# ExaScience/bpmf

Hardware: AMD Instinct MI355X
Metric: user+item column samples/sec per Gibbs iter; test RMSE vs reference (higher is better)
Workload: dtype f64

## Files before the change

bpmf_amd/csrc/kernels.h:

```cpp
#pragma once
#include <hip/hip_runtime.h>
#include <stdint.h>

#include "philox.h"
#include "args.h"

namespace bpmf {

typedef double d4 __attribute__((ext_vector_type(4)));

__device__ __forceinline__ d4 mfma16(double a, double b, d4 c)
{
    return __builtin_amdgcn_mfma_f64_16x16x4f64(a, b, c, 0, 0, 0);
}

__device__ __forceinline__ double mfma44(double a, double b, double c)
{
    return __builtin_amdgcn_mfma_f64_4x4x4f64(a, b, c, 0, 0, 0);
}

template <int K>
struct Rot44 {
    static constexpr int NT = K / 16;
    __host__ __device__ static constexpr int nrot(int TI, int TJ) { return TI == TJ ? 3 : 4; }
    __host__ __device__ static constexpr int aoff(int TI, int TJ)
    {
        int n = 0;
        for (int a = 0; a < NT; ++a)
            for (int b = a; b < NT; ++b) {
                if (a == TI && b == TJ) return n;
                n += nrot(a, b);
            }
        return n;
    }
    static constexpr int NACC = aoff(NT - 1, NT - 1) + 3;
};

template <int D>
__device__ __forceinline__ double quad_rot(double x)
{
    constexpr int CTRL = 0x120 + (16 - 4 * D);
    const long long v = __builtin_bit_cast(long long, x);
    const int lo = __builtin_amdgcn_update_dpp(0, (int)v, CTRL, 0xF, 0xF, true);
    const int hi = __builtin_amdgcn_update_dpp(0, (int)(v >> 32), CTRL, 0xF, 0xF, true);
    return __builtin_bit_cast(double, ((long long)hi << 32) | (unsigned int)lo);
}

template <int K>
__device__ __forceinline__ void rot44_contract(const double (&yy)[K / 16], double (&C)[Rot44<K>::NACC])
{
    using G = Rot44<K>;
    constexpr int NT = K / 16;
    double rot[NT][3];
#pragma unroll
    for (int t = 0; t < NT; ++t) {
        rot[t][0] = yy[t];
        rot[t][1] = quad_rot<1>(yy[t]);
        rot[t][2] = quad_rot<2>(yy[t]);
    }
#pragma unroll
    for (int TI = 0; TI < NT; ++TI)
#pragma unroll
        for (int TJ = TI; TJ < NT; ++TJ)
#pragma unroll
            for (int d = 0; d < G::nrot(TI, TJ); ++d) {
                if (d < 3) C[G::aoff(TI, TJ) + d] = mfma44(yy[TI], rot[TJ][d], C[G::aoff(TI, TJ) + d]);
                else C[G::aoff(TI, TJ) + d] = mfma44(rot[TI][1], yy[TJ], C[G::aoff(TI, TJ) + d]);
            }
}

template <int K, typename Sink>
__device__ __forceinline__ void rot44_images(const double (&C)[Rot44<K>::NACC], double *buf0, double *buf1, int lane, Sink &&sink)
{
    using G = Rot44<K>;
    constexpr int NT = G::NT;
    const int i = lane >> 4, b = (lane >> 2) & 3, j = lane & 3;
    int tix = 0;
#pragma unroll
    for (int TI = 0; TI < NT; ++TI)
#pragma unroll
        for (int TJ = TI; TJ < NT; ++TJ, ++tix) {
            double *img = (tix & 1) ? buf1 : buf0;
#pragma unroll
            for (int d = 0; d < G::nrot(TI, TJ); ++d) {
                const int row = d < 3 ? 4 * b + i : 4 * ((b + 1) & 3) + i, col = d < 3 ? 4 * ((b + d) & 3) + j : 4 * b + j;
                const double v = C[G::aoff(TI, TJ) + d];
                img[row * 16 + col] = v;
                if (TI == TJ && d > 0) img[col * 16 + row] = v;
            }
            __syncthreads();
#pragma unroll
            for (int m = 0; m < 4; ++m) sink(tix, TI, TJ, m, img[(4 * m + i) * 16 + (lane & 15)]);
            __syncthreads();
        }
}

__device__ __forceinline__ double rsqrt_nr(double d)
{
    const double y0 = __builtin_amdgcn_rsq(d);
    const double e = fma(-d, y0 * y0, 1.0);
    const double q = e * fma(0.375, e, 0.5);
    return fma(y0, q, y0);
}

__device__ __forceinline__ double gbcast(double v, int base_bytes, int off)
{
    const int lo = __builtin_amdgcn_ds_bpermute(base_bytes + 4 * off, __double2loint(v));
    const int hi = __builtin_amdgcn_ds_bpermute(base_bytes + 4 * off, __double2hiint(v));
    return __hiloint2double(hi, lo);
}

__device__ __forceinline__ double bcast(double v, int src)
{
    const int lo = __builtin_amdgcn_readlane(__double2loint(v), src);
    const int hi = __builtin_amdgcn_readlane(__double2hiint(v), src);
    return __hiloint2double(hi, lo);
}


__device__ __forceinline__ double polar_r2(double x, double y)
{
#pragma clang fp contract(off)
    return x * x + y * y;
}

__device__ __forceinline__ uint32_t sample_counter(int64_t idx, int ktrue, uint32_t iter_plus_1)
{
    return (uint32_t)((uint64_t)(idx + 1) * (uint64_t)ktrue * (uint64_t)iter_plus_1);
}

#define BPMF_RLX_SYSTEM_ __ATOMIC_RELAXED, __HIP_MEMORY_SCOPE_SYSTEM
enum { BPMF_TMO_GATE = 1, BPMF_TMO_PARAMS = 2, BPMF_TMO_STATS = 3 };
__device__ __forceinline__ void flag_timeout(unsigned long long *tmo, unsigned long long what)
{
    if (tmo) __hip_atomic_store(tmo, what, BPMF_RLX_SYSTEM_);
}

__device__ __forceinline__ void wait_params(const SampleArgs &a)
{
    if (a.gate_flag == nullptr) return;
    const unsigned long long t0 = wall_clock64();
    const unsigned long long limit = a.wait_ticks + (a.wait_ticks >> 1);
    while ((unsigned)__builtin_amdgcn_readfirstlane((int)__hip_atomic_load(a.gate_flag, __ATOMIC_RELAXED, __HIP_MEMORY_SCOPE_AGENT)) != a.gate_want) {
        __builtin_amdgcn_s_sleep(8);
        if (wall_clock64() - t0 > limit) {
            if (threadIdx.x == 0) flag_timeout(a.tmo, BPMF_TMO_PARAMS);
            break;
        }
    }
    asm volatile("" ::: "memory");
}

#ifndef BPMF_PROFILING
#define BPMF_PROFILING 0
#endif
constexpr bool kProfiling = BPMF_PROFILING != 0;
__device__ __forceinline__ uint32_t ablate_bits(const SampleArgs &a)
{
    if constexpr (kProfiling) return a.ablate;
    else return 0u;
}

__device__ __forceinline__ void stamp(const SampleArgs &a, int w, int slot)
{
    if constexpr (!kProfiling) {
        __builtin_amdgcn_sched_barrier(0);
        return;
    }
    if (a.stamps == nullptr || threadIdx.x != 0) return;
    const int probe = (w == 0) ? 0 : ((w == a.nwork / 2) ? 1 : -1);
    if (probe >= 0 && slot < 64) a.stamps[probe * 64 + slot] = wall_clock64();
}

__device__ __forceinline__ int rank_below(unsigned long long m)
{
    return (int)__builtin_amdgcn_mbcnt_hi((unsigned)(m >> 32), __builtin_amdgcn_mbcnt_lo((unsigned)m, 0u));
}

template <int NMAX>
__device__ __forceinline__ void draw_normals(uint32_t counter, int n, double *out_lds, int lane, int pad_to = 0)
{
    for (int i = n + lane; i < pad_to; i += 64) out_lds[i] = 0.0;
    int produced = 0;
    uint32_t base = 0;
    while (produced < n) {
        const Philox4 b = stream_block(counter, base + (uint32_t)lane);
        const double x = 2.0 * canonical53(b.w[3], b.w[2]) - 1.0;
        const double y = 2.0 * canonical53(b.w[1], b.w[0]) - 1.0;
        const double r2 = polar_r2(x, y);
        const bool acc = !(r2 > 1.0 || r2 == 0.0);
        const unsigned long long m = __ballot(acc);
        const int rank = produced + rank_below(m);
        if (acc && rank < n) {
            out_lds[rank] = y * polar_mult(r2);
        }
        produced += __popcll(m);
        base += 64u;
    }
}

template <int NMAX>
__device__ __forceinline__ void draw_normals_deferred(uint32_t counter, int n, double *out_lds, double *r2_lds, int lane, int pad_to = 0)
{
    for (int i = n + lane; i < pad_to; i += 64) out_lds[i] = 0.0;
    int produced = 0;
    uint32_t base = 0;
    while (produced < n) {
        const Philox4 b = stream_block(counter, base + (uint32_t)lane);
        const double x = 2.0 * canonical53(b.w[3], b.w[2]) - 1.0;
        const double y = 2.0 * canonical53(b.w[1], b.w[0]) - 1.0;
        const double r2 = polar_r2(x, y);
        const bool acc = !(r2 > 1.0 || r2 == 0.0);
        const unsigned long long m = __ballot(acc);
        const int rank = produced + rank_below(m);
        if (acc && rank < n) { out_lds[rank] = y; r2_lds[rank] = r2; }
        produced += __popcll(m);
        base += 64u;
    }
    for (int i = lane; i < n; i += 64) {
        const double r2 = r2_lds[i];
        out_lds[i] = out_lds[i] * polar_mult(r2);
    }
}

template <int NMAX>
__device__ __forceinline__ void draw_normals_pair(uint32_t counterA, uint32_t counterB, int n, double *outA, double *outB,
                                                  double *r2A, double *r2B, int lane, int pad_to = 0)
{
    for (int i = n + lane; i < pad_to; i += 64) { outA[i] = 0.0; outB[i] = 0.0; }
    auto attempt = [&](uint32_t counter, uint32_t block, double &y, double &r2) -> bool {
        const Philox4 b = stream_block(counter, block);
        const double x = 2.0 * canonical53(b.w[3], b.w[2]) - 1.0;
        y = 2.0 * canonical53(b.w[1], b.w[0]) - 1.0;
        r2 = polar_r2(x, y);
        return !(r2 > 1.0 || r2 == 0.0);
    };
    int prodA, prodB;
    {
        double y, r2;
        bool acc = attempt(counterA, (uint32_t)lane, y, r2);
        unsigned long long m = __ballot(acc);
        int rank = rank_below(m);
        if (acc && rank < n) { outA[rank] = y; r2A[rank] = r2; }
        prodA = __popcll(m);
        acc = attempt(counterB, (uint32_t)lane, y, r2);
        m = __ballot(acc);
        rank = rank_below(m);
        if (acc && rank < n) { outB[rank] = y; r2B[rank] = r2; }
        prodB = __popcll(m);
    }
    const bool hi = lane >= 32;
    const int l32 = lane & 31;
    uint32_t base = 64u;
    while (prodA < n || prodB < n) {
        double y, r2;
        const bool acc = attempt(hi ? counterB : counterA, base + (uint32_t)l32, y, r2);
        const unsigned long long m = __ballot(acc);
        const unsigned mA = (unsigned)m, mB = (unsigned)(m >> 32);
        const int rank = hi ? prodB + (int)__builtin_amdgcn_mbcnt_hi(mB, 0u) : prodA + (int)__builtin_amdgcn_mbcnt_lo(mA, 0u);
        if (acc && rank < n) { (hi ? outB : outA)[rank] = y; (hi ? r2B : r2A)[rank] = r2; }
        prodA += __popc(mA); prodB += __popc(mB);
        base += 32u;
    }
    for (int i = lane; i < n; i += 64) {
        const double ra = r2A[i], rb = r2B[i];
        outA[i] = outA[i] * polar_mult(ra);
        outB[i] = outB[i] * polar_mult(rb);
    }
}

template <int K>
__device__ __forceinline__ void gram_chunk(const int32_t *__restrict__ rowidx, const double *__restrict__ vals, int len,
                                           const double *__restrict__ other, const double *__restrict__ zero_row, double mean, double alpha,
                                           d4 (&acc)[Geo<K>::NTRI], double (&r)[Geo<K>::NT], int lane, int rowmask = -1)
{
    constexpr int NT = Geo<K>::NT;
    const int kq = lane >> 4, li = lane & 15;
    int ri_n = (0 + lane < len) ? rowidx[lane] : -1;
    double wv_n = (0 + lane < len) ? (vals[lane] - mean) * alpha : 0.0;
    for (int b = 0; b < len; b += 64) {
        const int ri = ri_n;
        const double wv = wv_n;
        if (b + 64 < len) {
            const int q = b + 64 + lane;
            ri_n = (q < len) ? rowidx[q] : -1;
            wv_n = (q < len) ? (vals[q] - mean) * alpha : 0.0;
        }
        const int nsteps = (len - b >= 64) ? 16 : (len - b + 3) >> 2;
        double y[4][NT], w[4];
        auto gather = [&](int g, double (&yy)[4][NT], double (&ww)[4]) {
#pragma unroll
            for (int s = 0; s < 4; ++s) {
                const int src = (g * 4 + s) * 4 + kq;
                const int row = __shfl(ri, src);
                ww[s] = __shfl(wv, src);
                const double *col = (row >= 0) ? other + (size_t)(row & rowmask) * K : zero_row;
#pragma unroll
                for (int t = 0; t < NT; ++t) yy[s][t] = col[(t * 16 + li < K) ? t * 16 + li : 0];
            }
        };
        gather(0, y, w);
#pragma unroll
        for (int g = 0; g < 4; ++g) {
            if (g * 4 >= nsteps) break;
            double yn[4][NT], wn[4];
// ... 658 lines not shown
            __hip_atomic_store(flag_host, seq, BPMF_RLX_SYSTEM);
        }
    }
}

template <int K>
constexpr bool kColstatsRot = (K == 64);

template <int K>
__device__ __forceinline__ void colstats_accumulate(const double *__restrict__ items, int64_t b, int64_t e,
                                                    d4 (&acc)[Geo<K>::NTRI], double (&r)[Geo<K>::NT], int lane, double *img,
                                                    const int32_t *__restrict__ list = nullptr, int64_t c0 = 0)
{
    constexpr int NT = Geo<K>::NT;
    constexpr bool ROT = kColstatsRot<K>;
    const int kq = lane >> 4, li = lane & 15;
    double C[ROT ? Rot44<K>::NACC : 1];
#pragma unroll
    for (int t = 0; t < (ROT ? Rot44<K>::NACC : 1); ++t) C[t] = 0.0;
#pragma unroll
    for (int t = 0; t < Geo<K>::NTRI; ++t) acc[t] = d4{0.0, 0.0, 0.0, 0.0};
#pragma unroll
    for (int t = 0; t < NT; ++t) r[t] = 0.0;
    double yn[2][NT];
    int64_t idn[2];
    auto ids = [&](int64_t c, int64_t (&id)[2]) {
#pragma unroll
        for (int s = 0; s < 2; ++s) {
            const int64_t pos = (c + s * 4 + kq < e) ? c + s * 4 + kq : b;
            id[s] = list ? c0 + (int64_t)list[pos] : pos;
        }
    };
    auto fetch = [&](const int64_t (&id)[2], double (&yy)[2][NT]) {
#pragma unroll
        for (int s = 0; s < 2; ++s) {
            const double *x = items + (size_t)id[s] * K;
#pragma unroll
            for (int t = 0; t < NT; ++t) yy[s][t] = x[(t * 16 + li < K) ? t * 16 + li : 0];
        }
    };
    if (b < e) {
        int64_t id0[2];
        ids(b, id0);
        fetch(id0, yn);
        ids((b + 8 < e) ? b + 8 : b, idn);
    }
    for (int64_t c = b; c < e; c += 8) {
        double y[2][NT];
#pragma unroll
        for (int s = 0; s < 2; ++s) {
            const bool ok = c + s * 4 + kq < e;
#pragma unroll
            for (int t = 0; t < NT; ++t) y[s][t] = (ok && (t * 16 + li < K)) ? yn[s][t] : 0.0;
        }
        fetch(idn, yn);
        ids((c + 16 < e) ? c + 16 : b, idn);
#pragma unroll
        for (int s = 0; s < 2; ++s) {
#pragma unroll
            for (int t = 0; t < NT; ++t) r[t] += y[s][t];
            if constexpr (ROT) {
                rot44_contract<K>(y[s], C);
            } else {
                int tri = 0;
#pragma unroll
                for (int I = 0; I < NT; ++I)
#pragma unroll
                    for (int J = I; J < NT; ++J, ++tri) acc[tri] = mfma16(y[s][I], y[s][J], acc[tri]);
            }
        }
    }
    if constexpr (ROT) rot44_images<K>(C, img, img + 256, lane, [&](int tix, int, int, int m, double v) { acc[tix][m] = v; });
#pragma unroll
    for (int t = 0; t < NT; ++t) {
        r[t] += __shfl_xor(r[t], 16);
        r[t] += __shfl_xor(r[t], 32);
    }
}

template <int K>
__device__ __forceinline__ void colstats_body(int w, const double *__restrict__ items, int64_t c0, int64_t c1, int nwaves,
                                              double *partials, const unsigned long long *__restrict__ fail_in,
                                              double *__restrict__ out, unsigned *ticket, unsigned *flag, unsigned seq,
                                              unsigned long long *tmo, unsigned long long wait_ticks, double *img)
{
    constexpr int NT = Geo<K>::NT, NTRI = Geo<K>::NTRI, PART = Geo<K>::PART;
    constexpr int NSUMS = blob::res_sums(K), NSLICE = (NSUMS + 15) / 16, FAILD = blob::res_failD(K), FAIL = blob::res_fail(K);
    const int lane = threadIdx.x;
    const int64_t n = c1 - c0;
    const int64_t per = (((n + nwaves - 1) / nwaves) + 3) & ~(int64_t)3;
    const int64_t b = c0 + w * per;
    const int64_t e = (b + per < c1) ? b + per : c1;

    {
        d4 acc[NTRI];
        double r[NT];
        colstats_accumulate<K>(items, b, e, acc, r, lane, img);
        double *p = partials + (size_t)w * PART;
#pragma unroll
        for (int t = 0; t < NTRI; ++t)
#pragma unroll
            for (int reg = 0; reg < 4; ++reg) __hip_atomic_store(&p[(t * 4 + reg) * 64 + lane], acc[t][reg], BPMF_RLX_AGENT);
        if (lane < 16) {
#pragma unroll
            for (int t = 0; t < NT; ++t) __hip_atomic_store(&p[NTRI * 256 + t * 16 + lane], r[t], BPMF_RLX_AGENT);
        }
    }

    const int nfin = nwaves < NSLICE ? nwaves : NSLICE;
    asm volatile("s_waitcnt vmcnt(0)" ::: "memory");
    unsigned tk = 0;
    if (lane == 0) tk = __hip_atomic_fetch_add(ticket, 1u, BPMF_RLX_AGENT);
    tk = __builtin_amdgcn_readfirstlane(tk);
    if ((int)tk < nwaves - nfin) return;
    const int f = (int)tk - (nwaves - nfin);
    if (lane == 0) {
        const unsigned long long t0 = wall_clock64();
        while (__hip_atomic_load(ticket, BPMF_RLX_AGENT) < (unsigned)nwaves) {
            __builtin_amdgcn_s_sleep(1);
            if (wait_ticks && wall_clock64() - t0 > wait_ticks) { flag_timeout(tmo, BPMF_TMO_STATS); break; }
        }
    }
    __syncthreads();

    const int o = lane & 15, grp = lane >> 4;
    for (int slice = f; slice < NSLICE; slice += nfin) {
        const int eo = slice * 16 + o;
        double s = 0.0;
        if (eo < NSUMS) {
            int off;
            if (eo < K * K) {
                int i = eo % K, j = eo / K;
                if (i > j) { const int t = i; i = j; j = t; }
                const int I = i >> 4, J = j >> 4;
                const int tri = I * NT - (I * (I - 1)) / 2 + (J - I);
                const int ii = i & 15, jj = j & 15;
                off = (tri * 4 + (ii >> 2)) * 64 + (ii & 3) * 16 + jj;
            } else {
                off = NTRI * 256 + (eo - K * K);
            }
            const int pw = (nwaves + 3) >> 2;
            const int w0 = grp * pw, w1 = (w0 + pw < nwaves) ? w0 + pw : nwaves;
            double acc[16];
#pragma unroll
            for (int u = 0; u < 16; ++u) acc[u] = 0.0;
            for (int ww = w0; ww < w1; ww += 16) {
                double v[16];
#pragma unroll
                for (int u = 0; u < 16; ++u)
                    v[u] = __hip_atomic_load(&partials[(size_t)((ww + u < w1) ? ww + u : w0) * PART + off], BPMF_RLX_AGENT);
#pragma unroll
                for (int u = 0; u < 16; ++u) acc[u] += (ww + u < w1) ? v[u] : 0.0;
            }
#pragma unroll
            for (int h = 8; h >= 1; h >>= 1)
#pragma unroll
                for (int u = 0; u < h; ++u) acc[u] += acc[u + h];
            s = acc[0];
        }
        s += __shfl_xor(s, 16);
        s += __shfl_xor(s, 32);
        if (grp == 0 && eo < NSUMS) __hip_atomic_store(&out[eo], s, BPMF_RLX_SYSTEM);
    }
    if (f == 0 && lane == 0) {
        const unsigned long long fw = __hip_atomic_load(fail_in, BPMF_RLX_AGENT);
        __hip_atomic_store(&out[FAILD], (fw == ~0ull) ? 0.0 : (double)(fw + 1ull), BPMF_RLX_SYSTEM);
        __hip_atomic_store(&reinterpret_cast<unsigned long long *>(out)[FAIL], fw, BPMF_RLX_SYSTEM);
    }
    publish_when_last(ticket + 1, (unsigned)nfin, flag, seq, ticket);
}

template <int K>
__global__ __launch_bounds__(64) void k_colstats(const double *__restrict__ items, int64_t c0, int64_t c1, int nwaves,
                                                 double *partials, const unsigned long long *__restrict__ fail_in,
                                                 double *__restrict__ out, unsigned *ticket, unsigned *flag, unsigned seq,
                                                 unsigned long long *tmo, unsigned long long wait_ticks)
{
    __shared__ double img[kColstatsRot<K> ? 512 : 1];
    colstats_body<K>((int)blockIdx.x, items, c0, c1, nwaves, partials, fail_in, out, ticket, flag, seq, tmo, wait_ticks, img);
}

template <int K>
__global__ __launch_bounds__(256) void k_colstats_wg(const double *__restrict__ items, int64_t c0, int64_t c1, int nwg,
                                                    double *partials, const unsigned long long *__restrict__ fail_in,
                                                    double *__restrict__ out, unsigned *ticket, unsigned *flag, unsigned seq,
                                                    unsigned long long *tmo, unsigned long long wait_ticks,
                                                    const int32_t *__restrict__ list, int part0, int ntot, int finish)
{
    constexpr int NT = Geo<K>::NT, NTRI = Geo<K>::NTRI, PART = Geo<K>::PART, NBLK = (PART + 63) / 64, FAILD = blob::res_failD(K), FAIL = blob::res_fail(K);
    __shared__ double red[PART];
    __shared__ double fin[4][64];
    __shared__ unsigned stk;
    const int tid = threadIdx.x, wave = tid >> 6, lane = tid & 63;
    const int64_t n = c1 - c0;
    const int nvw = nwg * 4, vw = (int)blockIdx.x * 4 + wave;
    const int64_t per = (((n + nvw - 1) / nvw) + 3) & ~(int64_t)3;
    const int64_t b = c0 + vw * per;
    const int64_t e = (b + per < c1) ? b + per : c1;
    {
        d4 acc[NTRI];
        double r[NT];
        static_assert(!kColstatsRot<K> || 4 * 512 <= PART, "the four waves' images fit the reduction buffer");
        colstats_accumulate<K>(items, b, e, acc, r, lane, red + 512 * wave, list, 0);
        if (kColstatsRot<K>) __syncthreads();
        for (int src = 1; src < 4; ++src) {
            if (wave == src) {
#pragma unroll
                for (int t = 0; t < NTRI; ++t)
#pragma unroll
                    for (int reg = 0; reg < 4; ++reg) red[(t * 4 + reg) * 64 + lane] = acc[t][reg];
                if (lane < 16) {
#pragma unroll
                    for (int t = 0; t < NT; ++t) red[NTRI * 256 + t * 16 + lane] = r[t];
                }
            }
            __syncthreads();
            if (wave == 0) {
#pragma unroll
                for (int t = 0; t < NTRI; ++t)
#pragma unroll
                    for (int reg = 0; reg < 4; ++reg) acc[t][reg] += red[(t * 4 + reg) * 64 + lane];
#pragma unroll
                for (int t = 0; t < NT; ++t) r[t] += red[NTRI * 256 + t * 16 + (lane & 15)];
            }
            __syncthreads();
        }
        if (wave == 0) {
            double *p = partials + (size_t)(part0 + (int)blockIdx.x) * PART;
#pragma unroll
            for (int t = 0; t < NTRI; ++t)
#pragma unroll
                for (int reg = 0; reg < 4; ++reg) __hip_atomic_store(&p[(t * 4 + reg) * 64 + lane], acc[t][reg], BPMF_RLX_AGENT);
            if (lane < 16) {
#pragma unroll
                for (int t = 0; t < NT; ++t) __hip_atomic_store(&p[NTRI * 256 + t * 16 + lane], r[t], BPMF_RLX_AGENT);
            }
            asm volatile("s_waitcnt vmcnt(0)" ::: "memory");
        }
    }
    if (!finish) return;
    const int nfin = nwg < NBLK ? nwg : NBLK;
    if (tid == 0) stk = __hip_atomic_fetch_add(ticket, 1u, BPMF_RLX_AGENT);
    __syncthreads();
    const unsigned tk = stk;
    if ((int)tk < nwg - nfin) return;
    const int f = (int)tk - (nwg - nfin);
    if (tid == 0) {
        const unsigned long long t0 = wall_clock64();
        while (__hip_atomic_load(ticket, BPMF_RLX_AGENT) < (unsigned)nwg) {
            __builtin_amdgcn_s_sleep(1);
            if (wait_ticks && wall_clock64() - t0 > wait_ticks) { flag_timeout(tmo, BPMF_TMO_STATS); break; }
        }
    }
    __syncthreads();
    const int pw = (ntot + 3) >> 2;
    const int w0 = wave * pw, w1 = (w0 + pw < ntot) ? w0 + pw : ntot;
    for (int blk = f; blk < NBLK; blk += nfin) {
        const int po = blk * 64 + lane;
        const int pc = po < PART ? po : 0;
        double acc[16];
#pragma unroll
        for (int u = 0; u < 16; ++u) acc[u] = 0.0;
        for (int ww = w0; ww < w1; ww += 16) {
            double v[16];
#pragma unroll
            for (int u = 0; u < 16; ++u)
                v[u] = __hip_atomic_load(&partials[(size_t)((ww + u < w1) ? ww + u : w0) * PART + pc], BPMF_RLX_AGENT);
#pragma unroll
            for (int u = 0; u < 16; ++u) acc[u] += (ww + u < w1) ? v[u] : 0.0;
        }
#pragma unroll
        for (int h = 8; h >= 1; h >>= 1)
#pragma unroll
            for (int u = 0; u < h; ++u) acc[u] += acc[u + h];
        fin[wave][lane] = acc[0];
        __syncthreads();
        if (wave == 0 && po < PART) {
            const double sum = ((fin[0][lane] + fin[1][lane]) + fin[2][lane]) + fin[3][lane];
            if (po < NTRI * 256) {
                const int tri = po >> 8, reg = (po >> 6) & 3, ln = po & 63;
                int I = 0, t = tri;
                while (t >= NT - I) { t -= NT - I; ++I; }
                const int J = I + t;
                const int gi = 16 * I + (ln >> 4) + 4 * reg, gj = 16 * J + (ln & 15);
                if (gi < K && gj < K) {
                    __hip_atomic_store(&out[gi + (size_t)gj * K], sum, BPMF_RLX_SYSTEM);
                    if (I != J) __hip_atomic_store(&out[gj + (size_t)gi * K], sum, BPMF_RLX_SYSTEM);
                }
            } else {
                const int el = po - NTRI * 256;
                if (el < K) __hip_atomic_store(&out[K * K + el], sum, BPMF_RLX_SYSTEM);
            }
        }
        __syncthreads();
    }
    if (f == 0 && tid == 0) {
        const unsigned long long fw = *fail_in;
        __hip_atomic_store(&out[FAILD], (fw == ~0ull) ? 0.0 : (double)(fw + 1ull), BPMF_RLX_SYSTEM);
        __hip_atomic_store(&reinterpret_cast<unsigned long long *>(out)[FAIL], fw, BPMF_RLX_SYSTEM);
    }
    publish_when_last(ticket + 1, (unsigned)nfin, flag, seq, ticket);
}

template <int K, int NT = 256, typename T = double>
__global__ __launch_bounds__(NT) void k_predict(const int32_t *__restrict__ tcol, const int32_t *__restrict__ trow,
                                                 const double *__restrict__ tval, int64_t nnz,
                                                 const T *__restrict__ items, const T *__restrict__ other,
                                                 int64_t col_from, double mean, int n, double *__restrict__ pavg,
                                                 double *__restrict__ pm2, double *partial, double *__restrict__ out,
                                                 unsigned *ticket, unsigned *flag, unsigned seq, TwinArgs tw)
{
    __shared__ double red[4][NT / 64];
    __shared__ double fin[4][NT];
    __shared__ unsigned last;
    auto wsum = [](const double (&r)[NT / 64]) { if constexpr (NT == 256) return (r[0] + r[1]) + (r[2] + r[3]); else return r[0]; };
    const int64_t q = (int64_t)blockIdx.x * NT + threadIdx.x;
    double se = 0.0, se_avg = 0.0, se_t = 0.0, se_avg_t = 0.0;
    if (q < nnz) {
        double d0 = 0.0, d1 = 0.0;
        if constexpr (sizeof(T) == 4) {
            const float4 *m = reinterpret_cast<const float4 *>(items + (size_t)(col_from + tcol[q]) * K);
            const float4 *u = reinterpret_cast<const float4 *>(other + (size_t)trow[q] * K);
#pragma unroll 8
            for (int t = 0; t < K / 4; ++t) {
                const float4 x = m[t], y = u[t];
                d0 = fma((double)x.x, (double)y.x, d0);
                d1 = fma((double)x.y, (double)y.y, d1);
                d0 = fma((double)x.z, (double)y.z, d0);
                d1 = fma((double)x.w, (double)y.w, d1);
            }
        } else {
            const double2 *m = reinterpret_cast<const double2 *>(items + (size_t)(col_from + tcol[q]) * K);
            const double2 *u = reinterpret_cast<const double2 *>(other + (size_t)trow[q] * K);
#pragma unroll
            for (int t = 0; t < K / 2; ++t) {
                const double2 a = m[t], b = u[t];
                d0 = fma(a.x, b.x, d0);
                d1 = fma(a.y, b.y, d1);
            }
        }
        const double pred = (d0 + d1) + mean;
        const double v = tval[q];
        se = (v - pred) * (v - pred);
        double avg = pavg[q];
        const double delta = pred - avg;
        avg = (n == 0) ? pred : (avg + delta / n);
        pavg[q] = avg;
        pm2[q] = (n == 0) ? 0.0 : pm2[q] + delta * (pred - avg);
        se_avg = (v - avg) * (v - avg);
        if (tw.perm) {
            const int qt = tw.perm[q];
            const double pred_t = (d0 + d1) + tw.mean;
            se_t = (v - pred_t) * (v - pred_t);
            double avg_t = tw.pavg[qt];
            const double delta_t = pred_t - avg_t;
            avg_t = (n == 0) ? pred_t : (avg_t + delta_t / n);
            tw.pavg[qt] = avg_t;
            tw.pm2[qt] = (n == 0) ? 0.0 : tw.pm2[qt] + delta_t * (pred_t - avg_t);
            se_avg_t = (v - avg_t) * (v - avg_t);
        }
    }
#pragma unroll
    for (int sh = 32; sh >= 1; sh >>= 1) {
        se += __shfl_xor(se, sh);
        se_avg += __shfl_xor(se_avg, sh);
        se_t += __shfl_xor(se_t, sh);
        se_avg_t += __shfl_xor(se_avg_t, sh);
    }
    const int wv = threadIdx.x >> 6;
    if ((threadIdx.x & 63) == 0) { red[0][wv] = se; red[1][wv] = se_avg; red[2][wv] = se_t; red[3][wv] = se_avg_t; }
    __syncthreads();
    if (threadIdx.x == 0) {
        __hip_atomic_store(&partial[2 * blockIdx.x], wsum(red[0]), BPMF_RLX_AGENT);
        __hip_atomic_store(&partial[2 * blockIdx.x + 1], wsum(red[1]), BPMF_RLX_AGENT);
        if (tw.perm) {
            __hip_atomic_store(&tw.partial[2 * blockIdx.x], wsum(red[2]), BPMF_RLX_AGENT);
            __hip_atomic_store(&tw.partial[2 * blockIdx.x + 1], wsum(red[3]), BPMF_RLX_AGENT);
        }
        asm volatile("s_waitcnt vmcnt(0)" ::: "memory");
        const unsigned t = __hip_atomic_fetch_add(ticket, 1u, BPMF_RLX_AGENT);
        last = (t == gridDim.x - 1) ? 1u : 0u;
    }
    __syncthreads();
    if (!last) return;
    {
        const int64_t nblocks = gridDim.x;
        double a = 0.0, b = 0.0, at = 0.0, bt = 0.0;
        for (int64_t w = threadIdx.x; w < nblocks; w += NT) {
            a += __hip_atomic_load(&partial[2 * w], BPMF_RLX_AGENT);
            b += __hip_atomic_load(&partial[2 * w + 1], BPMF_RLX_AGENT);
            if (tw.perm) {
                at += __hip_atomic_load(&tw.partial[2 * w], BPMF_RLX_AGENT);
                bt += __hip_atomic_load(&tw.partial[2 * w + 1], BPMF_RLX_AGENT);
            }
        }
        fin[0][threadIdx.x] = a; fin[1][threadIdx.x] = b; fin[2][threadIdx.x] = at; fin[3][threadIdx.x] = bt;
        __syncthreads();
        for (int st = NT / 2; st >= 1; st >>= 1) {
            if ((int)threadIdx.x < st) {
#pragma unroll
                for (int c = 0; c < 4; ++c) fin[c][threadIdx.x] += fin[c][threadIdx.x + st];
            }
            __syncthreads();
        }
        if (threadIdx.x == 0) {
            __hip_atomic_store(&out[0], fin[0][0], BPMF_RLX_SYSTEM);
            __hip_atomic_store(&out[1], fin[1][0], BPMF_RLX_SYSTEM);
            if (tw.perm) {
                __hip_atomic_store(&tw.out[0], fin[2][0], BPMF_RLX_SYSTEM);
                __hip_atomic_store(&tw.out[1], fin[3][0], BPMF_RLX_SYSTEM);
            }
            __hip_atomic_store(ticket, 0u, BPMF_RLX_AGENT);
            asm volatile("s_waitcnt vmcnt(0)" ::: "memory");
            __hip_atomic_store(flag, seq, BPMF_RLX_SYSTEM);
            if (tw.perm) __hip_atomic_store(tw.flag, tw.seq, BPMF_RLX_SYSTEM);
        }
    }
}

template <int K>
__global__ __launch_bounds__(256) void k_pack_cols(const double *__restrict__ items, const int32_t *__restrict__ cols, int64_t n,
                                                   double *__restrict__ buf)
{
    typedef double dd2 __attribute__((ext_vector_type(2)));
    constexpr int P = K / 2;
    const int64_t i = (int64_t)blockIdx.x * 256 + threadIdx.x;
    if (i >= n * P) return;
    const int64_t c = i / P;
    const int piece = (int)(i % P);
    reinterpret_cast<dd2 *>(buf)[i] = reinterpret_cast<const dd2 *>(items + (size_t)cols[c] * K)[piece];
}

template <int K>
__global__ __launch_bounds__(256) void k_unpack_cols(const double *__restrict__ buf, const int32_t *__restrict__ cols, int64_t n,
                                                     double *__restrict__ items)
{
    typedef double dd2 __attribute__((ext_vector_type(2)));
    constexpr int P = K / 2;
    const int64_t i = (int64_t)blockIdx.x * 256 + threadIdx.x;
    if (i >= n * P) return;
    const int64_t c = i / P;
    const int piece = (int)(i % P);
    reinterpret_cast<dd2 *>(items + (size_t)cols[c] * K)[piece] = reinterpret_cast<const dd2 *>(buf)[i];
}


__device__ __forceinline__ void gate_stage_body(int block, int nblocks, const unsigned *gate_host, unsigned want, const double *src_host,
                                                double *__restrict__ dst, int n, unsigned *dflag, unsigned dval,
                                                unsigned long long *tmo, unsigned long long wait_ticks)
{
    const int lane = threadIdx.x;
    if (lane == 0) {
        const unsigned long long t0 = wall_clock64();
        int polls = 0;
        while (__hip_atomic_load(gate_host, __ATOMIC_RELAXED, __HIP_MEMORY_SCOPE_SYSTEM) != want) {
            if (polls < 16) { __builtin_amdgcn_s_sleep(4); ++polls; }
            else __builtin_amdgcn_s_sleep(127);
            if (wall_clock64() - t0 > wait_ticks) { flag_timeout(tmo, BPMF_TMO_GATE); break; }
        }
        (void)__hip_atomic_load(gate_host, __ATOMIC_ACQUIRE, __HIP_MEMORY_SCOPE_SYSTEM);
    }
    __syncthreads();
    typedef double d2 __attribute__((ext_vector_type(2)));
    const d2 *src = reinterpret_cast<const d2 *>(src_host);
    d2 *out = reinterpret_cast<d2 *>(dst);
    const int n2 = n >> 1;
    for (int base = block * 256; base < n2; base += 256 * nblocks) {
        d2 v[4];
#pragma unroll
        for (int u = 0; u < 4; ++u) {
            const int i = base + u * 64 + lane;
            v[u] = (i < n2) ? __builtin_nontemporal_load(src + i) : d2{0.0, 0.0};
        }
#pragma unroll
        for (int u = 0; u < 4; ++u) {
            const int i = base + u * 64 + lane;
            if (i < n2) {
                if (dflag) {
                    __hip_atomic_store(dst + 2 * i, v[u].x, BPMF_RLX_AGENT);
                    __hip_atomic_store(dst + 2 * i + 1, v[u].y, BPMF_RLX_AGENT);
                } else {
                    out[i] = v[u];
                }
            }
        }
    }
    if (dflag) {
        asm volatile("s_waitcnt vmcnt(0)" ::: "memory");
        __syncthreads();
        if (lane == 0) __hip_atomic_store(dflag, dval, BPMF_RLX_AGENT);
    }
}



}
```

bpmf_amd/csrc/kernels_wg2.h:

```cpp
#pragma once
#include <type_traits>
#include "kernels_f32.h"
#include "kernels_slab.h"

namespace bpmf {

template <int B, int E, typename F>
__device__ __forceinline__ void static_for(F &&f)
{
    if constexpr (B < E) {
        f(std::integral_constant<int, B>{});
        static_for<B + 1, E>(f);
    }
}

template <int K>
struct GeoW2 {
    using F = GeoF<K>;
    static constexpr int NT = F::NT;
    template <typename T = float> static constexpr size_t lds_bytes() { return (size_t)K * 8 + ((size_t)F::RWORDS + K + 16 + 4) * sizeof(T); }
    static constexpr int PART_FLOATS = F::NTRI * 256 + NT * 16;
};

template <int NT, int NW>
struct FactOwner {
    static_assert(NT == 8 && (NW == 2 || NW == 4), "K = 128");
    __host__ __device__ static constexpr int of(int I, int J)
    {
        if (NW == 2) return 1;
        constexpr int tab[8][8] = {{0, 1, 3, 3, 2, 1, 2, 1}, {0, 1, 2, 1, 1, 2, 3, 3}, {0, 0, 2, 3, 1, 2, 1, 3}, {0, 0, 0, 3, 1, 2, 2, 3},
                                   {0, 0, 0, 0, 1, 2, 3, 1}, {0, 0, 0, 0, 0, 2, 3, 2}, {0, 0, 0, 0, 0, 0, 3, 1}, {0, 0, 0, 0, 0, 0, 0, 1}};
        return tab[I][J];
    }
    __host__ __device__ static constexpr int slot(int I, int J)
    {
        int n = 0;
        for (int i = 1; i < NT; ++i)
            for (int j = i; j < NT; ++j) {
                if (i == I && j == J) return n;
                if (of(i, j) == of(I, J)) ++n;
            }
        return n;
    }
    __host__ __device__ static constexpr int count(int W)
    {
        int n = 0;
        for (int i = 1; i < NT; ++i)
            for (int j = i; j < NT; ++j) n += of(i, j) == W;
        return n;
    }
    __host__ __device__ static constexpr int tiles() { int m = 0; for (int w = 1; w < NW; ++w) m = count(w) > m ? count(w) : m; return m; }
};

template <int MIDBAR = -1>
__device__ __forceinline__ void diag16_factor_invert(double (&A)[4], double (&E)[4], int lane)
{
    const int kq = lane >> 4, x = lane & 3, c16 = lane & 15;
    const W44Select wsel(kq, x);
#pragma unroll
    for (int I = 0; I < 4; ++I) E[I] = (4 * I + kq == c16) ? 1.0 : 0.0;
#pragma unroll
    for (int s = 0; s < 4; ++s) {
        const double dblk = A[s];
        const double d00 = bcast(dblk, 4 * s + 0), d01 = bcast(dblk, 4 * s + 1), d02 = bcast(dblk, 4 * s + 2), d03 = bcast(dblk, 4 * s + 3),
                     d11 = bcast(dblk, 16 + 4 * s + 1), d12 = bcast(dblk, 16 + 4 * s + 2), d13 = bcast(dblk, 16 + 4 * s + 3),
                     d22 = bcast(dblk, 32 + 4 * s + 2), d23 = bcast(dblk, 32 + 4 * s + 3), d33 = bcast(dblk, 48 + 4 * s + 3);
        double WA;
        factor_block44(d00, d01, d02, d03, d11, d12, d13, d22, d23, d33, wsel, WA);
        A[s] = mfma44(WA, A[s], 0.0);
        E[s] = mfma44(WA, E[s], 0.0);
        if (s == MIDBAR) __syncthreads();
        if (s == 3) break;
        double n1 = 0.0, n2 = 0.0, n3 = 0.0;
        if (s < 1) n1 = -quad_splat<1>(A[s]);
        if (s < 2) n2 = -quad_splat<2>(A[s]);
        n3 = -quad_splat<3>(A[s]);
        if (s < 1) { A[1] = mfma44(n1, A[s], A[1]); E[1] = mfma44(n1, E[s], E[1]); }
        if (s < 2) { A[2] = mfma44(n2, A[s], A[2]); E[2] = mfma44(n2, E[s], E[2]); }
        A[3] = mfma44(n3, A[s], A[3]); E[3] = mfma44(n3, E[s], E[3]);
    }
}

template <int K, int NW, int W, typename T = float>
__device__ __forceinline__ void wg2_column(const SampleArgs &a, int w, unsigned char *smem, int tid)
{
    using G = GeoF<K>;
    using X = WgTraits<T>;
    typedef typename X::acc_t acc_t;
    constexpr bool F32 = sizeof(T) == 4;
    constexpr int NT = G::NT, TPW = (G::NTRI + NW - 1) / NW;
    double *zs = reinterpret_cast<double *>(smem);
    T *R = reinterpret_cast<T *>(zs + K);
    T *bv = R + G::RWORDS, *xs = bv, *ts = bv + K;
    unsigned *sticket = reinterpret_cast<unsigned *>(ts + 16);
    const int lane = tid & 63;
    const int kq = lane >> 4, li = lane & 15;
    const int col = a.wi_col[w];
    const int64_t p0 = a.wi_p0[w];
    const int len = (ablate_bits(a) & 2u) ? 0 : a.wi_len[w];
    const int mc = a.wi_mc[w];
    const int64_t idx = a.col_from + col;
    const T *other = reinterpret_cast<const T *>(a.other_items);

    stamp(a, w, 0);

    acc_t acc[TPW];
    T r[NT];
#pragma unroll
    for (int t = 0; t < TPW; ++t) acc[t] = acc_t{0, 0, 0, 0};
#pragma unroll
    for (int t = 0; t < NT; ++t) r[t] = 0;
    const double *LF = a.prop_lambda ? a.prop_lambda + (size_t)col * K * K : a.LambdaF;
    bool lf_tiles = false;
    if constexpr (F32) lf_tiles = a.lf32 != nullptr;
    const double inv_alpha = 1.0 / a.alpha;
    auto prior = [&](auto firstc) {
        constexpr bool first = decltype(firstc)::value;
    if constexpr (F32) if (lf_tiles) {
        const f4 *lt = reinterpret_cast<const f4 *>(a.lf32);
        const T alpha_f = (T)a.alpha, inv_alpha_f = (T)(1.0 / a.alpha);
        f4 lf[TPW];
#pragma unroll
        for (int I = 0; I < NT; ++I)
#pragma unroll
            for (int J = I; J < NT; ++J)
                if ((G::tri(I, J) % NW) == W) lf[G::tri(I, J) / NW] = lt[G::tri(I, J) * 64 + lane];
#pragma unroll
        for (int I = 0; I < NT; ++I)
#pragma unroll
            for (int J = I; J < NT; ++J)
                if ((G::tri(I, J) % NW) == W) {
#pragma unroll
                    for (int reg = 0; reg < 4; ++reg) {
                        const T v = first ? lf[G::tri(I, J) / NW][reg] * inv_alpha_f : fmaf(alpha_f, acc[G::tri(I, J) / NW][reg], lf[G::tri(I, J) / NW][reg]);
                        acc[G::tri(I, J) / NW][reg] = (!first && a.diag_only && (16 * I + 4 * kq + reg) != (16 * J + li)) ? (T)0 : v;
                    }
                }
    }
    if (!lf_tiles) {
        constexpr int BATCH = first ? TPW : 6;
#pragma unroll
        for (int t0 = 0; t0 < TPW; t0 += BATCH) {
            double lf[BATCH][4];
#pragma unroll
            for (int u = 0; u < BATCH; ++u) {
                const int tri = (t0 + u) * NW + W;
                if (t0 + u < TPW && tri < G::NTRI) {
                    const int I = G::tile_i(tri), J = G::tile_j(tri);
#pragma unroll
                    for (int reg = 0; reg < 4; ++reg) lf[u][reg] = LF[(16 * J + li) + (size_t)(16 * I + X::drow(kq, reg)) * K];
                }
            }
#pragma unroll
            for (int u = 0; u < BATCH; ++u) {
                const int tri = (t0 + u) * NW + W;
                if (t0 + u < TPW && tri < G::NTRI) {
                    const int I = G::tile_i(tri), J = G::tile_j(tri);
#pragma unroll
                    for (int reg = 0; reg < 4; ++reg) {
                        const T v = first ? (T)(lf[u][reg] * inv_alpha) : (T)fma(a.alpha, (double)acc[t0 + u][reg], lf[u][reg]);
                        acc[t0 + u][reg] = (!first && a.diag_only && (16 * I + X::drow(kq, reg)) != (16 * J + li)) ? (T)0 : v;
                    }
                }
            }
        }
    }
    };
    const bool alpha_pow2 = a.alpha > 0.0 && (__double_as_longlong(a.alpha) & 0x000FFFFFFFFFFFFFll) == 0 &&
                            a.alpha >= 0x1p-500 && a.alpha <= 0x1p500;
    const bool whole = mc < 0 && alpha_pow2 && !lf_tiles;
    {
        const int32_t *rowidx = a.rowidx + p0;
        const double *vals = a.vals + p0;
        int ri = (lane < len) ? rowidx[lane] : -1;
        T wv = (lane < len) ? (T)((vals[lane] - a.mean_rating) * a.alpha) : (T)0;
        int ri_n = (64 + lane < len) ? rowidx[64 + lane] : -1;
        T wv_n = (64 + lane < len) ? (T)((vals[64 + lane] - a.mean_rating) * a.alpha) : (T)0;
        const int rowmask = (ablate_bits(a) & 4u) ? 63 : -1;
        const bool no_mfma = (ablate_bits(a) & 8u) != 0;
        constexpr int SPW = 4 / NW;
        constexpr int EPV = 16 / (int)sizeof(T), VPR = NT / EPV;
        typedef T tvec __attribute__((ext_vector_type(EPV)));
        constexpr int SBUF = 16 * K;
        static_assert(2 * SBUF <= G::RWORDS, "the staging buffers live where R will");
        T pre[SPW][NT];
        auto fetch = [&](int gg) {
            const bool nx = gg >= 4;
#pragma unroll
            for (int u = 0; u < SPW; ++u) {
                const int st = W + u * NW;
                const int src = ((gg & 3) * 4 + st) * 4 + kq;
                const int row = __shfl(nx ? ri_n : ri, src);
                const T *up = ((row >= 0) ? other + (size_t)(row & rowmask) * K : reinterpret_cast<const T *>(a.zero_row)) + li;
#pragma unroll
                for (int t = 0; t < NT; ++t) pre[u][t] = up[16 * t];
            }
        };
        auto stage = [&](int buf) {
#pragma unroll
            for (int u = 0; u < SPW; ++u) {
                const int st = W + u * NW;
#pragma unroll
                for (int v = 0; v < VPR; ++v) {
                    tvec x;
#pragma unroll
                    for (int e = 0; e < EPV; ++e) x[e] = pre[u][v * EPV + e];
                    reinterpret_cast<tvec *>(R + buf * SBUF)[(st * VPR + v) * 64 + lane] = x;
                }
            }
        };
        auto step = [&](int buf, int st, T w1) {
            T yy[NT];
#pragma unroll
            for (int v = 0; v < VPR; ++v) {
                const tvec x = reinterpret_cast<const tvec *>(R + buf * SBUF)[(st * VPR + v) * 64 + lane];
#pragma unroll
                for (int e = 0; e < EPV; ++e) yy[v * EPV + e] = x[e];
            }
            if (W == 0 || no_mfma) {
#pragma unroll
                for (int t = 0; t < NT; ++t) r[t] = fma(yy[t], w1, r[t]);
            }
            if (no_mfma) return;
#pragma unroll
            for (int I = 0; I < NT; ++I)
#pragma unroll
                for (int J = I; J < NT; ++J)
                    if ((G::tri(I, J) % NW) == W)
                        acc[G::tri(I, J) / NW] = X::mfma(yy[I], yy[J], acc[G::tri(I, J) / NW]);
        };
        const int ngr = (len + 15) >> 4;
        if (ngr > 0) fetch(0);
        if (whole) prior(std::true_type{});
        if (ngr > 0) stage(0);
        __syncthreads();
        for (int g = 0; g < ngr; ++g) {
            const int gl = g & 3;
            const bool more = g + 1 < ngr;
            if (more) fetch(gl + 1);
            T w1[4] = {0, 0, 0, 0};
            if (W == 0 || no_mfma) {
#pragma unroll
                for (int st = 0; st < 4; ++st) w1[st] = __shfl(wv, (gl * 4 + st) * 4 + kq);
            }
#pragma unroll
            for (int st = 0; st < 4; ++st) step(g & 1, st, w1[st]);
            if (more) stage((g + 1) & 1);
            if (gl == 3) {
                ri = ri_n; wv = wv_n;
                const int q = (g >> 2) * 64 + 128 + lane;
                ri_n = (q < len) ? rowidx[q] : -1;
                wv_n = (q < len) ? (T)((vals[q] - a.mean_rating) * a.alpha) : (T)0;
            }
            __syncthreads();
        }
        if (W == 0) {
#pragma unroll
            for (int t = 0; t < NT; ++t) {
                r[t] += __shfl_xor(r[t], 16);
                r[t] += __shfl_xor(r[t], 32);
            }
        }
    }

    __builtin_amdgcn_s_setprio(3);
    stamp(a, w, 1);
    if (kProfiling && W == 1 && a.stamps && lane == 0 && (w == 0 || w == a.nwork / 2)) a.stamps[(w == 0 ? 0 : 64) + 48] = wall_clock64();
    if (mc >= 0) {
        constexpr int PF = GeoW2<K>::PART_FLOATS;
        const int nch = a.mc_nchunks[mc];
        T *pbase = reinterpret_cast<T *>(a.partials) + (size_t)a.mc_slot0[mc] * PF;
        T *p = pbase + (size_t)a.wi_chunk[w] * PF;
#pragma unroll
        for (int I = 0; I < NT; ++I)
#pragma unroll
            for (int J = I; J < NT; ++J)
                if ((G::tri(I, J) % NW) == W) {
#pragma unroll
                    for (int reg = 0; reg < 4; ++reg) __hip_atomic_store(&p[G::tri(I, J) * 256 + reg * 64 + lane], acc[G::tri(I, J) / NW][reg], BPMF_RLX_AGENT);
                }
        if (W == 0 && lane < 16) {
#pragma unroll
            for (int t = 0; t < NT; ++t) __hip_atomic_store(&p[G::NTRI * 256 + t * 16 + lane], r[t], BPMF_RLX_AGENT);
        }
        asm volatile("s_waitcnt vmcnt(0)" ::: "memory");
        __syncthreads();
        if (tid == 0) *sticket = __hip_atomic_fetch_add(&a.mc_count[mc], 1u, BPMF_RLX_AGENT);
        __syncthreads();
        const unsigned tk = *sticket;
        if ((int)tk != nch - 1) return;
        if (tid == 0) __hip_atomic_store(&a.mc_count[mc], 0u, BPMF_RLX_AGENT);
#pragma unroll
        for (int t = 0; t < TPW; ++t) acc[t] = acc_t{0, 0, 0, 0};
#pragma unroll
        for (int t = 0; t < NT; ++t) r[t] = 0;
        for (int ch = 0; ch < nch; ++ch) {
            const T *pc = pbase + (size_t)ch * PF;
#pragma unroll
            for (int I = 0; I < NT; ++I)
#pragma unroll
                for (int J = I; J < NT; ++J)
                    if ((G::tri(I, J) % NW) == W) {
#pragma unroll
                        for (int reg = 0; reg < 4; ++reg) acc[G::tri(I, J) / NW][reg] += __hip_atomic_load(&pc[G::tri(I, J) * 256 + reg * 64 + lane], BPMF_RLX_AGENT);
                    }
            if (W == 0) {
#pragma unroll
                for (int t = 0; t < NT; ++t) r[t] += __hip_atomic_load(&pc[G::NTRI * 256 + t * 16 + li], BPMF_RLX_AGENT);
            }
        }
    }

    if (ablate_bits(a) & 1u) {
        T v = r[0];
#pragma unroll
        for (int t = 0; t < TPW; ++t) v += acc[t][0] + acc[t][1] + acc[t][2] + acc[t][3];
        if (lane < 16) reinterpret_cast<T *>(a.items)[(size_t)idx * K + 16 * W + lane] = v;
// ... 272 lines not shown
```

Baseline: 104.9 million.

## Cooperative coalesced f64 dot products in predict kernel via lane groups and swizzle reduction

Replaces the per-thread strided row loads in the f64 prediction kernel with a cooperative scheme. Groups of up to 16 lanes share row indices via ds_swizzle, and each group loads contiguous double2 chunks of one row pair at a time. Partial sums are then reduced with an XOR-swizzle butterfly so each lane ends up with its own dot product. This is meant to coalesce memory accesses to the item/user factor rows, at the cost of extra cross-lane swizzle ops and register arrays.

```diff
diff --git a/bpmf_amd/csrc/kernels.h b/bpmf_amd/csrc/kernels.h
--- a/bpmf_amd/csrc/kernels.h
+++ b/bpmf_amd/csrc/kernels.h
@@ -1,6 +1,7 @@
 #pragma once
 #include <hip/hip_runtime.h>
 #include <stdint.h>
+#include <type_traits>
 
 #include "philox.h"
 #include "args.h"
@@ -1265,6 +1266,37 @@
     publish_when_last(ticket + 1, (unsigned)nfin, flag, seq, ticket);
 }
 
+template <int B, int E, typename F>
+__device__ __forceinline__ void static_for(F &&f)
+{
+    if constexpr (B < E) {
+        f(std::integral_constant<int, B>{});
+        static_for<B + 1, E>(f);
+    }
+}
+
+template <int AND, int OR, int XOR>
+__device__ __forceinline__ int swizzle(int v) { return __builtin_amdgcn_ds_swizzle(v, (AND & 31) | (OR << 5) | (XOR << 10)); }
+template <int H>
+__device__ __forceinline__ double swizzle_xor(double v)
+{
+    const long long w = __double_as_longlong(v);
+    const unsigned lo = (unsigned)swizzle<31, 0, H>((int)(unsigned)w), hi = (unsigned)swizzle<31, 0, H>((int)(unsigned)(w >> 32));
+    return __longlong_as_double((long long)(((unsigned long long)hi << 32) | lo));
+}
+
+template <int H, int N>
+__device__ __forceinline__ void predict_halve(double (&s)[N], int p)
+{
+    const bool up = (p & H) != 0;
+    static_for<0, H>([&](auto ic) {
+        constexpr int i = decltype(ic)::value;
+        const double keep = up ? s[i + H] : s[i], give = up ? s[i] : s[i + H];
+        s[i] = keep + swizzle_xor<H>(give);
+    });
+    if constexpr (H > 2) predict_halve<H / 2>(s, p);
+}
+
 template <int K, int NT = 256, typename T = double>
 __global__ __launch_bounds__(NT) void k_predict(const int32_t *__restrict__ tcol, const int32_t *__restrict__ trow,
                                                  const double *__restrict__ tval, int64_t nnz,
@@ -1279,8 +1311,42 @@
     auto wsum = [](const double (&r)[NT / 64]) { if constexpr (NT == 256) return (r[0] + r[1]) + (r[2] + r[3]); else return r[0]; };
     const int64_t q = (int64_t)blockIdx.x * NT + threadIdx.x;
     double se = 0.0, se_avg = 0.0, se_t = 0.0, se_avg_t = 0.0;
+    double d0 = 0.0, d1 = 0.0;
+    if constexpr (sizeof(T) == 8) {
+        constexpr int P = K / 2, LPE = P < 16 ? P : 16, R = P / LPE;
+        constexpr int RB = (16 / R < LPE) ? 16 / R : LPE;
+        const int64_t q0 = q - (int64_t)(threadIdx.x & 63);
+        if (q0 < nnz) {
+            const int p = (int)(threadIdx.x & (LPE - 1));
+            const int64_t qc = q < nnz ? q : nnz - 1;
+            const int mi = (int)(col_from + tcol[qc]), ui = trow[qc];
+            double s[LPE];
+            static_for<0, LPE / RB>([&](auto bc) {
+                constexpr int rb = decltype(bc)::value * RB;
+                double2 a[RB][R], b[RB][R];
+                static_for<0, RB>([&](auto rc) {
+                    constexpr int r = decltype(rc)::value;
+                    const double2 *m = reinterpret_cast<const double2 *>(items + (size_t)swizzle<~(LPE - 1), rb + r, 0>(mi) * K) + p;
+                    const double2 *u = reinterpret_cast<const double2 *>(other + (size_t)swizzle<~(LPE - 1), rb + r, 0>(ui) * K) + p;
+#pragma unroll
+                    for (int j = 0; j < R; ++j) { a[r][j] = m[LPE * j]; b[r][j] = u[LPE * j]; }
+                });
+                __builtin_amdgcn_sched_barrier(0);
+#pragma unroll
+                for (int r = 0; r < RB; ++r) {
+                    double acc = 0.0;
+#pragma unroll
+                    for (int j = 0; j < R; ++j) acc = fma(a[r][j].y, b[r][j].y, fma(a[r][j].x, b[r][j].x, acc));
+                    s[rb + r] = acc;
+                }
+            });
+            predict_halve<LPE / 2>(s, p);
+            const bool up = (p & 1) != 0;
+            d0 = up ? s[1] : s[0];
+            d1 = swizzle_xor<1>(up ? s[0] : s[1]);
+        }
+    }
     if (q < nnz) {
-        double d0 = 0.0, d1 = 0.0;
         if constexpr (sizeof(T) == 4) {
             const float4 *m = reinterpret_cast<const float4 *>(items + (size_t)(col_from + tcol[q]) * K);
             const float4 *u = reinterpret_cast<const float4 *>(other + (size_t)trow[q] * K);
@@ -1291,15 +1357,6 @@
                 d1 = fma((double)x.y, (double)y.y, d1);
                 d0 = fma((double)x.z, (double)y.z, d0);
                 d1 = fma((double)x.w, (double)y.w, d1);
-            }
-        } else {
-            const double2 *m = reinterpret_cast<const double2 *>(items + (size_t)(col_from + tcol[q]) * K);
-            const double2 *u = reinterpret_cast<const double2 *>(other + (size_t)trow[q] * K);
-#pragma unroll
-            for (int t = 0; t < K / 2; ++t) {
-                const double2 a = m[t], b = u[t];
-                d0 = fma(a.x, b.x, d0);
-                d1 = fma(a.y, b.y, d1);
             }
         }
         const double pred = (d0 + d1) + mean;
diff --git a/bpmf_amd/csrc/kernels_wg2.h b/bpmf_amd/csrc/kernels_wg2.h
--- a/bpmf_amd/csrc/kernels_wg2.h
+++ b/bpmf_amd/csrc/kernels_wg2.h
@@ -5,14 +5,6 @@
 
 namespace bpmf {
 
-template <int B, int E, typename F>
-__device__ __forceinline__ void static_for(F &&f)
-{
-    if constexpr (B < E) {
-        f(std::integral_constant<int, B>{});
-        static_for<B + 1, E>(f);
-    }
-}
 
 template <int K>
 struct GeoW2 {
```

New measurement: 106.6 million (median of 6 runs). Within noise of the previous version (+1.6%).
